# LuletterSoul/RP-Style-Transfer

Measured on AMD Instinct MI355X. Metric: stylized images/sec at 512×512, 1/2/4/8 MI355X; % HBM roofline, higher is better.
Workload: dtype fp32

## Files before the change

### rp-style-transfer_amd/csrc/rpst_conv.h

```cpp
#pragma once

#include "rpst_common.h"

namespace rpst {

constexpr int kTW = 32;

struct ConvArgs {
  const float* in;
  const float* aux;
  const float* aux2;
  const float* wpk;
  const float* bias;
  const float* res;
  float* out;
  int N, Cin, Hs, Ws, H, W, Cout, Cout_pad, nchunks;
  int tiles_x, tiles_y, co_tiles;
  int pad, relu;
  int persist;
  int cosplit;
  float2* stat_part;
  int stat_P;
  int64_t wstride;
  const float* btab;
  int skip_from;
  const float* in2;
  int in2_from;
  const float* mask;
  int pool_out;
};

struct ConvMode {
  int precise;
  int quarter;
  int algo;
  bool narrow;
  int narrow_rpt;
};

struct ConvTiling {
  int64_t blocks;
  int nth;
  int stat_nt, stat_wn, stat_tw;
  bool stat_t;
};

__device__ __forceinline__ const float* conv_in_img(const ConvArgs& a, int n, int64_t per) {
  return (a.in2_from > 0 && n >= a.in2_from) ? a.in2 + (int64_t)(n - a.in2_from) * per
                                             : a.in + (int64_t)n * per;
}

template <int KS>
struct ConvK {
  static constexpr int CK = (KS == 3) ? 8 : 16;
  static constexpr int TAPS = KS * KS;
  static constexpr int KCH = TAPS * CK;
};

__device__ __forceinline__ bool resolve(int& v, int n, int pad, bool padded) {
  if (padded) {
    if (pad == RPST_PAD_ZERO) {
      if (v < 0 || v >= n) return false;
    } else {
      v = reflect1(v, n);
    }
  }
  v = v < 0 ? 0 : (v >= n ? n - 1 : v);
// ... 167 lines not shown
  v += __builtin_bit_cast(float, __builtin_amdgcn_update_dpp(0, __builtin_bit_cast(int, v), 0xB1, 0xF, 0xF, false));
  v += __builtin_bit_cast(float, __builtin_amdgcn_update_dpp(0, __builtin_bit_cast(int, v), 0x4E, 0xF, 0xF, false));
  v += __builtin_bit_cast(float, __builtin_amdgcn_update_dpp(0, __builtin_bit_cast(int, v), 0x141, 0xF, 0xF, false));
  v += __builtin_bit_cast(float, __builtin_amdgcn_update_dpp(0, __builtin_bit_cast(int, v), 0x140, 0xF, 0xF, false));
  return v;
}
__device__ __forceinline__ bool resolve_bf(int& v, int n, bool zero_pad) {
  const bool in = v >= 0 && v < n;
  const int r = reflect1(v, n);
  v = zero_pad ? min(max(v, 0), n - 1) : r;
  return in || !zero_pad;
}
__device__ __forceinline__ void at6(const float (&m)[6], float (&p)[4]) {
  const float s12 = m[1] + m[2], d12 = m[1] - m[2];
  const float s34 = m[3] + m[4], d34 = m[3] - m[4];
  p[0] = (m[0] + s12) + s34;
  p[1] = fmaf(2.f, d34, d12);
  p[2] = fmaf(4.f, s34, s12);
  p[3] = fmaf(8.f, d34, d12) + m[5];
}
__device__ __forceinline__ void w4_tile(int b, int tiles_x, int tiles_y, int& tx, int& ty, int& n) {
  ty = b % tiles_y;
  b /= tiles_y;
  tx = b % tiles_x;
  n = b / tiles_x;
}

bool wino4q_applies(int Cin, int Cout, int in_op, const ConvMode& m);
size_t wino4q_packed_floats(int Cout, int Cin);
int wino4q_pack(const float* w, float* pk, int Cout, int Cin, hipStream_t st);
int wino4q_pack_mix(const double* wm, float* pk, int N, int Cout, int Cin, hipStream_t st);
int wino4q_fold_w(const float* pk, float* out, const float* aux, int N, int Cout, int Cin,
                  hipStream_t st);
ConvTiling wino4q_tiling(ConvArgs& a);
int wino4q_launch(ConvArgs& a, int in_op, hipStream_t st);
inline size_t wino4_image_floats(int Cout, int Cin, bool quarter) {
  return quarter ? wino4q_packed_floats(Cout, Cin) : wino4_packed_floats(Cout, Cin);
}
inline size_t wino4_image_floats_max(int Cout, int Cin) {
  const size_t q = wino4q_packed_floats(Cout, Cin), p = wino4_packed_floats(Cout, Cin);
  return q > p ? q : p;
}

}
```

### rp-style-transfer_amd/csrc/rpst_conv.hip

```cpp
#include "rpst_conv.h"

#include <cstdlib>
#include <cstring>

namespace rpst {

template <int KS, int BM, int TH, int WM, int WN, int INOP, int NTH, int CKK, bool DB>
__global__ __launch_bounds__(NTH, 2) void conv_mfma_kernel(ConvArgs a) {
  using K = ConvK<KS>;
  constexpr int PCK = K::CK, TAPS = K::TAPS;
  constexpr int CK = CKK, KCH = TAPS * CK;
  static_assert(PCK % CK == 0, "kernel chunk must divide the packing chunk");
  constexpr int OFF = (KS == 3) ? 1 : 0;
  constexpr int PH = TH + KS - 1, PW = kTW + KS - 1;
  constexpr int WTM = BM / WM;
  constexpr int MT = WTM / 32;
  constexpr int NT = TH / WN;
  static_assert(WM * WN == NTH / kWave, "one wave per sub-tile");
  static_assert(MT >= 1 && NT >= 1 && (CK % 2) == 0, "tile");
  constexpr int NW4 = KCH * BM / 4;
  constexpr int WLD = (NW4 + NTH - 1) / NTH;
  constexpr bool WFULL = (NW4 % NTH) == 0;
  constexpr int GROUPS = NTH / 32;
  constexpr int CPT = CK > GROUPS ? CK / GROUPS : 1;
// ... 500 lines not shown
  const int wn = bm == 128 ? 2 : 4;
  a.Cout_pad = pad_cout(a.Cout);
  a.nchunks = (a.Cin + ck - 1) / ck;
  a.tiles_x = (a.W + kTW - 1) / kTW;
  a.tiles_y = (a.H + th - 1) / th;
  a.co_tiles = a.Cout_pad / bm;
  a.stat_P = a.tiles_x * a.tiles_y * wn;
  return {(int64_t)a.tiles_x * a.tiles_y * a.N * a.co_tiles, 256, th / wn, wn, kTW, false};
}

static int narrow_rpt(int Cout, const ConvMode& m) {
  return Cout <= 4 && m.narrow_rpt != 2 ? 4 : 2;
}
static ConvTiling narrow_tiling(ConvArgs& a, int rpt) {
  const int rows = 4 * rpt;
  a.Cout_pad = pad_cout(a.Cout);
  a.nchunks = (a.Cin + ConvK<3>::CK - 1) / ConvK<3>::CK;
  a.tiles_x = (a.W + kNrTW - 1) / kNrTW;
  a.tiles_y = (a.H + rows - 1) / rows;
  a.co_tiles = 1;
  a.stat_P = 0;
  return {(int64_t)a.tiles_x * a.tiles_y * a.N, 256, 0, 0, kNrTW, false};
}

static thread_local int t_conv_precise = 0;
static thread_local int t_conv_quarter = -1;

static ConvMode conv_mode() {
  ConvMode m{};
  m.precise = t_conv_precise;
  const char* e = getenv("RPST_W4Q");
  const int q = t_conv_quarter >= 0 ? t_conv_quarter : ((e && *e) ? atoi(e) : 1);
  m.quarter = q == 2 ? 2 : q != 0;
  e = getenv("RPST_CONV_ALGO");
  m.algo = -1;
  if (e && e[0] == 'd') m.algo = RPST_CONV_DIRECT;
  else if (e && !strcmp(e, "winograd")) m.algo = RPST_CONV_WINOGRAD;
  else if (e && !strcmp(e, "winograd4")) m.algo = RPST_CONV_WINOGRAD4;
  e = getenv("RPST_CONV_NARROW");
  m.narrow = !(e && *e && atoi(e) == 0);
  e = getenv("RPST_CONV_NARROW_RPT");
  m.narrow_rpt = (e && *e && atoi(e) == 2) ? 2 : 0;
  return m;
}

static int conv_algo(int Cout, int Cin, int Hs, int Ws, int ksize, int in_op, const ConvMode& m) {
  if (ksize != 3) return RPST_CONV_DIRECT;
  const bool w4 = wino4_supports(in_op) && wino4_fits(1, Cin, Hs, Ws, in_op);
  const bool nr = (in_op == RPST_IN_NONE || (in_op == RPST_IN_ADD_ADAIN && Cout <= 4)) &&
                  narrow_shape(Cin, Cout) && m.narrow;
  if (m.algo == RPST_CONV_DIRECT) return nr ? RPST_CONV_NARROW : RPST_CONV_DIRECT;
  if (m.algo == RPST_CONV_WINOGRAD) return RPST_CONV_WINOGRAD;
  if (m.algo == RPST_CONV_WINOGRAD4) return w4 ? RPST_CONV_WINOGRAD4 : RPST_CONV_WINOGRAD;
  if (nr) return RPST_CONV_NARROW;
  if (Cin <= 4 && w4 && m.precise != 1) return RPST_CONV_WINOGRAD4;
  if (Cin < 16) return RPST_CONV_DIRECT;
  if (w4 && m.precise != 1) return RPST_CONV_WINOGRAD4;
  if (w4) return RPST_CONV_WINOGRAD;
  return Cout >= 32 ? RPST_CONV_WINOGRAD : RPST_CONV_DIRECT;
}

static size_t direct_packed_floats(int Cout, int Cin, int ksize) {
  const int ck = ck_of(ksize);
  const size_t nch = (size_t)(Cin + ck - 1) / ck;
  return nch * ksize * ksize * ck * (size_t)pad_cout(Cout);
}
// ... 16 lines not shown
}

struct ConvNeeds {
  bool stats, residual, fold;
};

struct ConvPlan {
  int algo;
  bool quarter;
  bool fold;
  int op;
  int rpt;
  size_t wofs;
  ConvTiling t;
};

static ConvPlan conv_plan(ConvArgs& a, int ksize, int in_op, const ConvMode& m, ConvNeeds need) {
  ConvPlan p{};
  p.op = in_op;
  p.algo = conv_algo(a.Cout, a.Cin, a.Hs, a.Ws, ksize, in_op, m);
  if (p.algo == RPST_CONV_NARROW) {
    p.rpt = narrow_rpt(a.Cout, m);
    p.t = narrow_tiling(a, p.rpt);
    if (need.stats || a.N > 65535 || a.tiles_y > 65535) p.algo = RPST_CONV_DIRECT;
  }
  if (need.residual && (p.algo == RPST_CONV_WINOGRAD || p.algo == RPST_CONV_WINOGRAD4))
    p.algo = RPST_CONV_DIRECT;
  if (p.algo == RPST_CONV_WINOGRAD4) {
    p.fold = need.fold && !need.stats && a.H >= 2 && a.W >= 2;
    if (p.fold) p.op = RPST_IN_NONE;
    p.quarter = wino4q_applies(a.Cin, a.Cout, p.op, m);
    p.wofs = direct_packed_floats(a.Cout, a.Cin, ksize) + wino_packed_floats(a.Cout, a.Cin) +
             (p.quarter ? wino4_packed_floats(a.Cout, a.Cin) : 0);
    p.t = p.quarter ? wino4q_tiling(a) : wino4_tiling(a);
  } else if (p.algo == RPST_CONV_WINOGRAD) {
    p.wofs = direct_packed_floats(a.Cout, a.Cin, ksize);
    p.t = wino_tiling(a, in_op);
  } else if (p.algo == RPST_CONV_DIRECT) {
    p.t = direct_tiling(a, ksize, in_op);
  }
  return p;
}

template <class F>
static size_t max_over_modes(ConvMode m, F bytes) {
  size_t best = 0;
  for (m.precise = 0; m.precise < 3; ++m.precise)
    for (m.quarter = 0; m.quarter < 3; ++m.quarter) {
      const size_t b = bytes(m);
      best = b > best ? b : best;
    }
  return best;
}

}

using namespace rpst;

extern "C" size_t rpst_conv2d_packed_size(int Cout, int Cin, int ksize) {
  if (Cout <= 0 || Cin <= 0 || (ksize != 1 && ksize != 3)) return 0;
  size_t f = direct_packed_floats(Cout, Cin, ksize);
  if (ksize == 3)
    f += wino_packed_floats(Cout, Cin) + wino4_packed_floats(Cout, Cin) +
         wino4q_packed_floats(Cout, Cin);
  return f * sizeof(float);
}

// ... 124 lines not shown
  a.mask = r.mask;
  a.pool_out = r.pool_out;
  if (r.ksize == 3 && r.pad_mode == RPST_PAD_REFLECT)
    RPST_REQUIRE(a.H >= 2 && a.W >= 2, "conv2d: reflect padding needs H,W >= 2");
  RPST_REQUIRE((int64_t)r.N * (r.Cout > r.Cin ? r.Cout : r.Cin) * a.H * a.W < (1LL << 40),
               "conv2d: tensor too large");
  RPST_REQUIRE(((int64_t)r.Cin + 16) * r.Hs * r.Ws * 4 < (1LL << 31),
               "conv2d: one image's input exceeds 2 GiB");
  const bool fold = r.fold_ws && (r.in_op == RPST_IN_ADAIN || r.T);
  p = conv_plan(a, r.ksize, r.in_op, m, {r.stat_part != nullptr, r.residual != nullptr, fold});
  RPST_REQUIRE(!r.pool_out || p.algo == RPST_CONV_WINOGRAD4,
               "conv2d_pool: the pooled-output epilogue exists on the F(4x4) path only "
               "(rpst_conv2d_algorithm == RPST_CONV_WINOGRAD4)");
  RPST_REQUIRE(!r.T || p.fold, "conv2d_mix: T / offset on a launch that does not fold them");
  a.wpk = r.packed_weight + p.wofs;
  return RPST_OK;
}

template <int KS, int INOP>
static int launch_direct(const ConvArgs& a, hipStream_t st) {
  launch_conv<KS, INOP>(a, direct_bm(a.Cout), st);
  return launch_status("conv_mfma_kernel");
}

static int conv_launch(const ConvReq& r, ConvArgs& a, const ConvPlan& p) {
  hipStream_t st = r.st;
  if (p.algo == RPST_CONV_WINOGRAD4) {
    if (p.fold) {
      const int e = r.T ? wino4_mix(a, p.quarter, r.T, r.offset, r.packed_weight,
                                    pad_cout(r.Cout), r.fold_ws, st)
                        : wino4_fold(a, p.quarter, r.packed_weight, pad_cout(r.Cout), r.fold_ws, st);
      if (e) return e;
    }
    if (int e = p.quarter ? wino4q_launch(a, p.op, st) : wino4_launch(a, p.op, st)) return e;
    if (r.mask) {
      const int64_t n = (int64_t)r.N * r.Cout * a.H * a.W;
      mask_apply_kernel<<<(unsigned)((n + 1023) / 1024), 256, 0, st>>>(r.out, r.mask, n);
      return launch_status("mask_apply_kernel");
    }
    return RPST_OK;
  }
  if (p.algo == RPST_CONV_WINOGRAD) return wino_launch(a, r.in_op, st);
  if (p.algo == RPST_CONV_NARROW) {
    RPST_REQUIRE(r.Cin * 9 * (r.Cout <= 4 ? 4 : 16) <= kNrWl, "conv2d: narrow weights exceed LDS");
    const dim3 grid((unsigned)a.tiles_x, (unsigned)a.tiles_y, r.N);
    if (r.in_op == RPST_IN_ADD_ADAIN) {
      RPST_REQUIRE(r.Cout <= 4, "conv2d: narrow skip-AdaIN conv needs Cout <= 4");
      if (p.rpt == 4) conv3x3_narrow_kernel<4, 4, RPST_IN_ADD_ADAIN><<<grid, 256, 0, st>>>(a);
      else conv3x3_narrow_kernel<4, 2, RPST_IN_ADD_ADAIN><<<grid, 256, 0, st>>>(a);
    } else if (r.Cout <= 4) {
      if (p.rpt == 4) conv3x3_narrow_kernel<4, 4><<<grid, 256, 0, st>>>(a);
      else conv3x3_narrow_kernel<4, 2><<<grid, 256, 0, st>>>(a);
    } else {
      conv3x3_narrow_kernel<16, 2><<<grid, 256, 0, st>>>(a);
    }
    return launch_status("conv3x3_narrow_kernel");
  }
  RPST_REQUIRE(p.t.blocks <= 0x7fffffffLL, "conv2d: grid too large");
  if (r.ksize == 1) {
    RPST_REQUIRE(r.in_op == RPST_IN_NONE, "conv2d: 1x1 conv supports in_op NONE only");
    return launch_direct<1, RPST_IN_NONE>(a, st);
  }
  switch (r.in_op) {
    case RPST_IN_MAXPOOL2: return launch_direct<3, RPST_IN_MAXPOOL2>(a, st);
    case RPST_IN_UPSAMPLE2: return launch_direct<3, RPST_IN_UPSAMPLE2>(a, st);
    case RPST_IN_ADD_UPSAMPLE2: return launch_direct<3, RPST_IN_ADD_UPSAMPLE2>(a, st);
    case RPST_IN_ADAIN: return launch_direct<3, RPST_IN_ADAIN>(a, st);
// ... 315 lines not shown
```

### rp-style-transfer_amd/csrc/rpst_wino4q.hip

```cpp
#include "rpst_conv.h"

#include <type_traits>

#ifndef RPST_W4Q_DBG
#define RPST_W4Q_DBG 0
#endif

namespace rpst {
namespace {

template <int PAD>
__device__ __forceinline__ void q_mfma(floatx4& acc, float a, float b) {
  if constexpr (PAD)
    asm volatile("s_nop 1\n\tv_mfma_f32_16x16x4_f32 %0, %1, %2, %0" : "+v"(acc) : "v"(a), "v"(b));
  else
    asm volatile("v_mfma_f32_16x16x4_f32 %0, %1, %2, %0" : "+v"(acc) : "v"(a), "v"(b));
}
__device__ __forceinline__ unsigned q_lds_addr(const float* p) {
  return (unsigned)(uintptr_t)(const __attribute__((address_space(3))) float*)p;
}
template <int OFF>
__device__ __forceinline__ void q_dma16(__amdgpu_buffer_rsrc_t r, unsigned m0, unsigned voff,
                                        int soff) {
  asm volatile("s_mov_b32 m0, %0\n\ts_nop 0\n\tbuffer_load_dwordx4 %1, %2, %3 offen offset:%4 lds"
// ... 14 lines not shown
                                      float& u0, float& u1, float& u2) {
  if constexpr (H == 0) {
    const float A = fmaf(-4.f, d2, d4), B = fmaf(-4.f, d1, d3);
    u0 = fmaf(4.f, d0, fmaf(-5.f, d2, d4));
    u1 = A + B;
    u2 = A - B;
  } else {
    const float C = d4 - d2, E = d3 - d1;
    u0 = fmaf(2.f, E, C);
    u1 = fmaf(-2.f, E, C);
    u2 = fmaf(4.f, d1, fmaf(-5.f, d3, d5));
  }
}

}

constexpr int kQCo = 64;
constexpr int kQTH = 8, kQTW = 64;
constexpr int kQXO = 4;
constexpr int kQPS = 72;
constexpr int kQCS = 768;
constexpr int kQWS = 9216;
constexpr int kQPAT = 4 * kQCS;
constexpr int kQNTH = 512;
constexpr int kQMaxCo = 512;
constexpr int kQWPI = 5;
constexpr int kQWide = 2, kQSlow = 6;
constexpr int kQDMA4 = 3, kQDMA = 12;
constexpr int kQRP = kQPS / 4;
constexpr int kQXS = 4 * 3 * 3 * 64 * 2;
constexpr int kQWG0 = 0;
constexpr int kQPG = 5;
constexpr int kQAhead = 3;
static_assert(10 * kQRP <= kQDMA4 * 64 && kQDMA4 * 256 <= kQCS, "16-B pieces in a channel");
static_assert(10 * kQPS <= kQDMA * 64 && kQDMA * 64 <= kQCS, "4-B pieces in a channel");
static_assert(2 * kQWide >= kQDMA4 && 2 * kQSlow >= kQDMA && 8 * kQWPI >= 36, "coverage");
static_assert(2 * kQXS <= kQWS, "the exchange fits a weight stage");
static_assert((2 * kQWS + 4 * kQPAT) * 4 + 1024 + kQSlow * kQNTH * 4 + 9 * kQMaxCo * 4 <= 163840,
              "LDS");

template <typename TW>
__global__ void wino4q_pack_kernel(const TW* __restrict__ w, float* __restrict__ pk, int Cout,
                                   int Cin, int K4, int64_t per, int64_t total, int64_t sco,
                                   int64_t sci, int64_t stap) {
  int64_t t = (int64_t)blockIdx.x * blockDim.x + threadIdx.x;
  if (t >= total) return;
  const int64_t img = t / per;
  pk += img * per;
  w += img * (int64_t)Cout * Cin * 9;
  t -= img * per;
  const int cb = (int)(t & 3);
  int64_t r = t >> 2;
  const int l = (int)(r & 63);
  r >>= 6;
  const int p = (int)(r % 9);
  r /= 9;
  const int q = (int)(r & 3);
  r >>= 2;
  const int ks = (int)(r % K4);
  const int ct = (int)(r / K4);
  const int i = 3 * (q >> 1) + p / 3, jj = 3 * (q & 1) + p % 3;
  const int co = ct * kQCo + cb * 16 + (l & 15);
  const int ci = ks * 4 + (l >> 4);
  float v = 0.f;
  if (co < Cout && ci < Cin) {
    const double G[6][3] = {{0.25, 0, 0},
// ... 33 lines not shown

__global__ void wino4q_fold_w_kernel(const float4* __restrict__ pk, float4* __restrict__ out,
                                     const float* __restrict__ aux, int N, int Cin, int K4,
                                     int64_t per4) {
  const int64_t t = (int64_t)blockIdx.x * blockDim.x + threadIdx.x;
  if (t >= (int64_t)N * per4) return;
  const int n = (int)(t / per4);
  const int64_t u = t - (int64_t)n * per4;
  const int l = (int)(u & 63);
  const int ks = (int)((u / (kQWS / 4)) % K4);
  const int ci = ks * 4 + (l >> 4);
  const int64_t nc = (int64_t)N * Cin, i = (int64_t)n * Cin + (ci < Cin ? ci : 0);
  const float sc = ci < Cin ? aux[3 * nc + i] / aux[2 * nc + i] : 0.f;
  const float4 v = pk[u];
  out[t] = make_float4(v.x * sc, v.y * sc, v.z * sc, v.w * sc);
}

int wino4q_fold_w(const float* pk, float* out, const float* aux, int N, int Cout, int Cin,
                  hipStream_t st) {
  const int64_t per4 = (int64_t)wino4q_packed_floats(Cout, Cin) / 4, n4 = (int64_t)N * per4;
  wino4q_fold_w_kernel<<<(unsigned)((n4 + 255) / 256), 256, 0, st>>>(
      reinterpret_cast<const float4*>(pk), reinterpret_cast<float4*>(out), aux, N, Cin,
      (Cin + 3) / 4, per4);
  return launch_status("wino4q_fold_w_kernel");
}

bool wino4q_applies(int Cin, int Cout, int in_op, const ConvMode& m) {
  const int min_cin = m.quarter == 2 ? 16 : 128;
  return m.quarter && m.precise != 2 && (in_op == RPST_IN_NONE || in_op == RPST_IN_UPSAMPLE2) &&
         Cout >= 64 && Cout <= kQMaxCo &&
         Cin >= min_cin && Cin % 16 == 0;
}

ConvTiling wino4q_tiling(ConvArgs& a) {
  a.Cout_pad = (a.Cout + kQCo - 1) / kQCo * kQCo;
  a.nchunks = (a.Cin + 3) / 4;
  a.tiles_x = (a.W + kQTW - 1) / kQTW;
  a.tiles_y = (a.H + kQTH - 1) / kQTH;
  a.co_tiles = a.Cout_pad / kQCo;
  a.stat_P = a.tiles_x * a.tiles_y * 2;
  a.cosplit = 1;
  return {(int64_t)a.tiles_x * a.tiles_y * a.N, kQNTH, 4, kQTH / 4, kQTW, true};
}

struct QEpi {
  int W, H, Cout, gy0, gx0, rows, n, sidx;
  bool vec, full, bst, edge, store, pool;
  float inv, slope;
  unsigned voff[4];
  float* out;
  float* oimg;
  unsigned obytes;
  const float* btab;
  float2* statp;
  int statP;
};

__device__ __forceinline__ QEpi q_epi_ctx(int wr, int tn) {
  const KArgs L = late_args();
  QEpi e;
  e.W = L->W;
  e.H = L->H;
  e.Cout = L->Cout;
  e.slope = L->relu == RPST_ACT_RELU ? 0.f : (L->relu == RPST_ACT_LRELU ? 0.2f : 1.f);
  int btx, bty;
  w4_tile((int)blockIdx.x / L->cosplit, L->tiles_x, L->tiles_y, btx, bty, e.n);
  const int bx0 = btx * kQTW;
  e.gy0 = bty * kQTH + 4 * wr;
  e.gx0 = bx0 + 4 * tn;
  e.vec = (e.W & 3) == 0 && e.gx0 + 3 < e.W;
  e.rows = max(0, min(4, e.H - e.gy0));
  const int cols = max(0, min(kQTW, e.W - bx0));
  e.inv = e.rows * cols > 0 ? __builtin_amdgcn_rcpf((float)(e.rows * cols)) : 0.f;
  e.full = e.rows == 4 && bx0 + kQTW <= e.W;
  e.edge = e.gy0 == 0 || e.gy0 + 4 >= e.H || bx0 == 0 || bx0 + kQTW >= e.W;
  e.out = L->out;
  const int64_t plane = (int64_t)e.H * e.W;
  e.pool = L->pool_out != 0;
  e.bst = !e.pool && (e.W & 3) == 0 && (int64_t)e.Cout * plane * 4 < (1LL << 31);
  e.oimg = e.out + (int64_t)e.n * e.Cout * plane;
  const bool keep = L->skip_from <= 0 || e.n < L->skip_from;
  e.obytes = keep ? (unsigned)(e.Cout * plane * 4) : 0u;
  e.store = keep;
#pragma unroll
  for (int yy = 0; yy < 4; ++yy)
    e.voff[yy] = (yy < e.rows && e.gx0 < e.W) ? (unsigned)(((e.gy0 + yy) * e.W + e.gx0) * 4)
                                             : 0x80000000u;
  e.btab = L->btab;
  e.statp = L->stat_part;
  e.statP = L->stat_P;
  e.sidx = (bty * L->tiles_x + btx) * 2 + wr;
  return e;
}

template <bool STATS, bool BTAB, bool RELU>
__device__ __forceinline__ void q_finish(const QEpi& e, int co, float (&Y)[16], int tn) {
  const int gy0 = e.gy0, gx0 = e.gx0, rows = e.rows, n = e.n;
  const bool cok = co < e.Cout;
  if constexpr (BTAB) {
// ... 96 lines not shown
#pragma unroll
      for (int i = 0; i < 16; ++i) m2 = fmaf(Y[i] - mean, Y[i] - mean, m2);
    } else {
#pragma unroll
      for (int yy = 0; yy < 4; ++yy)
#pragma unroll
        for (int xx = 0; xx < 4; ++xx) {
          const float dv = Y[yy * 4 + xx] - mean;
          m2 += (yy < rows && gx0 + xx < e.W) ? dv * dv : 0.f;
        }
    }
    m2 = row16_sum(m2);
    if (tn == 0 && cok)
      e.statp[((int64_t)n * e.statP + e.sidx) * e.Cout + co] = make_float2(mean, m2);
  }
}

template <int INOP, bool STATS, bool BTAB, bool RELU>
__global__ __launch_bounds__(kQNTH, 1) void wino4q_mfma_kernel(ConvArgs a) {
  __shared__ __attribute__((aligned(16))) float ws0[kQWS];
  __shared__ __attribute__((aligned(16))) float ws1[kQWS];
  __shared__ __attribute__((aligned(16))) float ps0[kQPAT];
  __shared__ __attribute__((aligned(16))) float ps1[kQPAT];
  __shared__ __attribute__((aligned(16))) float ps2[kQPAT];
  __shared__ __attribute__((aligned(16))) float ps3[kQPAT];
  __shared__ __attribute__((aligned(16))) float dummy[256];
  __shared__ unsigned poffs[kQSlow][kQNTH];
  __shared__ float btl[BTAB ? 9 * kQMaxCo : kQMaxCo];

  const int wave = __builtin_amdgcn_readfirstlane((int)threadIdx.x >> 6);
  const int lane = threadIdx.x & 63;
  const int k = lane >> 4, tn = lane & 15, wr = wave >> 2;

  int bid = (int)blockIdx.x;
  const int cog = bid % a.cosplit;
  bid /= a.cosplit;
  const int nct = a.co_tiles / a.cosplit, ct0 = cog * nct;
  int tx, ty, n;
  w4_tile(bid, a.tiles_x, a.tiles_y, tx, ty, n);
  const int K4 = a.nchunks, G = nct * K4;
  const int y0 = ty * kQTH, x0 = tx * kQTW;

  {
    const int nb = BTAB ? 9 * a.Cout : a.Cout;
    const float* src = BTAB ? a.btab + (int64_t)n * nb : a.bias;
    for (int i = threadIdx.x; i < nb; i += kQNTH) btl[i] = src ? src[i] : 0.f;
  }
  constexpr bool up = INOP == RPST_IN_UPSAMPLE2;
  const unsigned in_plane = up ? (unsigned)(a.Hs * a.Ws) : (unsigned)(a.H * a.W);
  const unsigned oob = a.Cin * in_plane * 4u;
  const float* in_img = conv_in_img(a, n, (int64_t)a.Cin * in_plane);
  const unsigned wbytes = (unsigned)(nct * K4 * kQWS) * 4u;
  const float* w_img = a.wpk + (int64_t)n * a.wstride + (int64_t)ct0 * K4 * kQWS;

  const int hf = wave & 1;
  const bool zp = a.pad == RPST_PAD_ZERO;
  const int rs = up ? a.Ws : a.W;
  const bool w4a = (a.W & 3) == 0;
  const bool wide = !up && ((x0 >= 1 && x0 + kQTW < a.W) || (w4a && x0 + kQTW <= a.W));
  const bool fixL = wide && w4a && !zp && x0 == 0;
  const bool fixR = wide && w4a && !zp && x0 + kQTW == a.W;
  unsigned poff[kQSlow];
  const int tid = threadIdx.x;
  if (wide) {
#pragma unroll
    for (int i = 0; i < kQWide; ++i) {
      const int p = kQWide * hf + i;
      const int f = 64 * p + lane, row = min(f / kQRP, 9), j = f - (f / kQRP) * kQRP;
      int y = y0 - 1 + row;
      const int xs = x0 - kQXO + 4 * j;
      const bool okx = !w4a || (xs >= 0 && xs + 3 < a.W);
      const bool ok = p < kQDMA4 && f < 10 * kQRP && resolve_bf(y, a.H, zp) && okx;
      poff[i] = ok ? ((unsigned)(y * rs) + (unsigned)xs) * 4u : oob;
    }
#pragma unroll
    for (int i = kQWide; i < kQSlow; ++i) poff[i] = oob;
  } else {
#pragma unroll
    for (int i = 0; i < kQSlow; ++i) {
      const int p = kQSlow * hf + i;
      const int f = 64 * p + lane;
      const int row = min(f / kQPS, 9), col = f - (f / kQPS) * kQPS;
      int y = y0 - 1 + row, x = x0 - kQXO + col;
      const bool oky = resolve_bf(y, a.H, zp), okx = resolve_bf(x, a.W, zp);
      const bool ok = p < kQDMA && col >= kQXO - 1 && col < kQXO + 1 + kQTW &&
                      f < 10 * kQPS && oky && okx;
      poff[i] = ok ? ((unsigned)((up ? y >> 1 : y) * rs) + (unsigned)(up ? x >> 1 : x)) * 4u : oob;
    }
  }
#pragma unroll
  for (int i = 0; i < kQSlow; ++i) poffs[i][tid] = poff[i];

  constexpr int DBG = RPST_W4Q_DBG;
  const int wl = wave * 4096;
  const bool real4 = wave < 4;
  const int w4 = 32768 + wave * 1024;
  const unsigned dummy_a = q_lds_addr(dummy);
  int wso = wl;
  auto issue_w = [&](bool live, unsigned stg, auto Ic) {
    constexpr int I = decltype(Ic)::value;
    if (DBG & 2) return;
    if constexpr (I < 4) {
      q_dma16<1024 * I>(rsrc_or_zero(w_img, wbytes, live), stg + wl, lane * 16, wso);
    } else {
      q_dma16<0>(rsrc_or_zero(w_img, wbytes, live && real4), real4 ? stg + w4 : dummy_a,
                 lane * 16, wso + (w4 - wl));
    }
  };
  const unsigned pstep = 4u * in_plane * 4u;
  const int pbase = (int)((unsigned)(wave >> 1) * in_plane * 4u);
  const bool h1 = (wave & 1) != 0;
  const int pl = (wave >> 1) * (kQCS * 4) + (h1 ? (wide ? 2048 : kQSlow * 256) : 0);
  int pso = pbase;
  auto issue_p = [&](auto WIDEc, bool live, unsigned stg) {
    constexpr bool WIDE = decltype(WIDEc)::value;
    if (DBG & 1) return;
    const auto r = rsrc_or_zero(in_img, oob, live);
    const unsigned xs = stg + launder(pl);
    if constexpr (WIDE) {
      q_dma16<0>(r, xs, poffs[0][tid], pso);
      q_dma16<0>(r, h1 ? dummy_a : xs + 1024, poffs[1][tid], pso);
    } else {
#pragma unroll
      for (int i = 0; i < kQSlow; ++i) q_dma4(r, xs + 256 * i, poffs[i][tid], pso);
    }
    pso += (int)pstep;
  };
  const bool bst_all = !a.pool_out && (a.W & 3) == 0 &&
                       (int64_t)a.Cout * a.H * a.W * 4 < (1LL << 31);
  bool post_epi = false;
  auto wait_ring = [&](bool first) {
    if (DBG & 128) return;
    if (first && post_epi && bst_all) {
      if (wide) asm volatile("s_waitcnt vmcnt(18)" ::: "memory");
      else asm volatile("s_waitcnt vmcnt(22)" ::: "memory");
    } else if (wide) {
      asm volatile("s_waitcnt vmcnt(2)" ::: "memory");
    } else {
      asm volatile("s_waitcnt vmcnt(6)" ::: "memory");
    }
    if (first) post_epi = false;
  };

  auto fix_halo = [&](float* stg) {
    if ((wave == 0 && fixL) || (wave == 1 && fixR)) {
      int l = lane;
      asm volatile("" : "+v"(l));
      if (l < 40) {
        const int ch = l / 10, row = l - 10 * ch;
        float* rp = stg + ch * kQCS + row * kQPS;
        if (wave == 0) rp[kQXO - 1] = rp[kQXO + 1];
        else rp[kQXO + kQTW] = rp[kQXO + kQTW - 2];
      }
    }
  };
  auto prologue = [&](auto WIDEc) {
    issue_p(WIDEc, true, q_lds_addr(ps0));
    issue_p(WIDEc, true, q_lds_addr(ps1));
    issue_w(true, q_lds_addr(ws0), std::integral_constant<int, 0>{});
    issue_w(true, q_lds_addr(ws0), std::integral_constant<int, 1>{});
    issue_w(true, q_lds_addr(ws0), std::integral_constant<int, 2>{});
    issue_w(true, q_lds_addr(ws0), std::integral_constant<int, 3>{});
    issue_w(true, q_lds_addr(ws0), std::integral_constant<int, 4>{});
    issue_p(WIDEc, true, q_lds_addr(ps2));
    issue_p(WIDEc, true, q_lds_addr(ps3));
  };
  if (wide) prologue(std::true_type{});
  else prologue(std::false_type{});
  wait_ring(false);
  q_lds_barrier();
  if (fixL || fixR) {
    fix_halo(ps0);
    fix_halo(ps1);
    q_lds_barrier();
  }

  auto body = [&](auto Qc) {
    constexpr int Q = decltype(Qc)::value, QR = Q >> 1, QC = Q & 1;
    floatx4 acc[9][4];
#pragma unroll
    for (int p = 0; p < 9; ++p)
#pragma unroll
      for (int cb = 0; cb < 4; ++cb) acc[p][cb] = floatx4{0.f, 0.f, 0.f, 0.f};
    const int roff = k * kQCS + (4 * wr + QR) * kQPS + 4 * tn;
    auto read_row = [&](const float* stg, int rr, float (&d)[8]) {
      const float* rp = stg + roff + rr * kQPS;
      floatx4 u = *reinterpret_cast<const floatx4*>(rp + 4);
      const float e = QC ? rp[8] : rp[3];
      asm("" : "+v"(u));
      d[0] = QC ? 0.f : e; d[1] = u[0]; d[2] = u[1]; d[3] = u[2]; d[4] = u[3];
      d[5] = QC ? e : 0.f; d[6] = 0.f; d[7] = 0.f;
    };
    auto col_pass = [&](const float (&d)[8], float (&u)[3]) {
      if (DBG & 8) {
        u[0] = d[0]; u[1] = d[1]; u[2] = d[2];
        return;
      }
      q_bt3<QC>(d[0], d[1], d[2], d[3], d[4], d[5], u[0], u[1], u[2]);
    };
    auto row_pass = [&](const float (&u)[5][3], int j, float (&v)[9]) {
      if (DBG & 8) {
        v[j] = u[0][j]; v[3 + j] = u[2][j]; v[6 + j] = u[4][j];
        return;
      }
      if constexpr (QR == 0)
        q_bt3<0>(u[0][j], u[1][j], u[2][j], u[3][j], u[4][j], 0.f, v[j], v[3 + j], v[6 + j]);
      else
        q_bt3<1>(0.f, u[0][j], u[1][j], u[2][j], u[3][j], u[4][j], v[j], v[3 + j], v[6 + j]);
    };
    float V[9];
    {
      float u[5][3];
#pragma unroll
      for (int rr = 0; rr < 5; ++rr) {
        float d[8];
        read_row(ps0, rr, d);
        col_pass(d, u[rr]);
      }
#pragma unroll
      for (int j = 0; j < 3; ++j) row_pass(u, j, V);
    }

    const int woff = Q * 9 * 256 + lane * 4;
    int x = 0;
    auto step = [&](float* wsx, float* psn, float* wsn, float* psx, float* pfx, int ks,
                    bool first) {
      wait_ring(first);
      const bool wlive = x + 1 < G, plive = x + 4 < G;
      wso += kQWS * 4;
      if (first && ks + 4 == K4) pso = pbase;
      const unsigned wsn_a = q_lds_addr(wsn), psx_a = q_lds_addr(psx);
      if (DBG & 16) asm volatile("s_waitcnt lgkmcnt(0)" ::: "memory");
      else q_lds_barrier();
      constexpr int ord[9] = {0, 3, 6, 1, 4, 7, 2, 5, 8};
      constexpr int kA = kQAhead;
      float4 w4[9];
#pragma unroll
      for (int q = 0; q < kA; ++q)
        w4[ord[q]] = *reinterpret_cast<const float4*>(wsx + woff + ord[q] * 256);
      float d[8];
      read_row(psn, 0, d);
      float u[5][3];
#pragma unroll
      for (int q = 0; q < 9; ++q) {
        const int p = ord[q];
        if (q + kA < 9)
          w4[ord[q + kA]] = *reinterpret_cast<const float4*>(wsx + woff + ord[q + kA] * 256);
        q_mfma<1>(acc[p][0], w4[p].x, V[p]);
        q_mfma<0>(acc[p][1], w4[p].y, V[p]);
        q_mfma<0>(acc[p][2], w4[p].z, V[p]);
        q_mfma<0>(acc[p][3], w4[p].w, V[p]);
        if (q == kQWG0) issue_w(wlive, wsn_a, std::integral_constant<int, 0>{});
        if (q == kQWG0 + 1) issue_w(wlive, wsn_a, std::integral_constant<int, 1>{});
        if (q == kQWG0 + 2) issue_w(wlive, wsn_a, std::integral_constant<int, 2>{});
        if (q == kQWG0 + 3) issue_w(wlive, wsn_a, std::integral_constant<int, 3>{});
        if (q == kQWG0 + 4) issue_w(wlive, wsn_a, std::integral_constant<int, 4>{});
        if (q == kQPG) {
          if (wide) issue_p(std::true_type{}, plive, psx_a);
          else issue_p(std::false_type{}, plive, psx_a);
        }
        if (q < 5) {
          col_pass(d, u[q]);
          if (q + 1 < 5) read_row(psn, q + 1, d);
        }
        if (q == 5 || q == 6 || q == 8) row_pass(u, q == 8 ? 2 : q - 5, V);
        if (q == 7) fix_halo(pfx);
      }
      ++x;
    };

    auto epilogue = [&](int ctile) {
      if (DBG & 32) {
        float t = 0.f;
#pragma unroll
        for (int p = 0; p < 9; ++p)
#pragma unroll
          for (int cb = 0; cb < 4; ++cb) t += acc[p][cb][0];
        if (t == 1.2345f) late_args()->out[threadIdx.x] = t;
#pragma unroll
        for (int p = 0; p < 9; ++p)
#pragma unroll
          for (int cb = 0; cb < 4; ++cb) acc[p][cb] = floatx4{0.f, 0.f, 0.f, 0.f};
        return;
      }
      q_lds_barrier();
      asm volatile("s_nop 7\n\ts_nop 4" : "+v"(acc[0][0]), "+v"(acc[0][1]), "+v"(acc[0][2]),
                   "+v"(acc[0][3]), "+v"(acc[1][0]), "+v"(acc[1][1]), "+v"(acc[1][2]),
                   "+v"(acc[1][3]), "+v"(acc[2][0]), "+v"(acc[2][1]), "+v"(acc[2][2]),
                   "+v"(acc[2][3]), "+v"(acc[3][0]), "+v"(acc[3][1]), "+v"(acc[3][2]),
                   "+v"(acc[3][3]), "+v"(acc[4][0]), "+v"(acc[4][1]));
      asm volatile("" : "+v"(acc[4][2]), "+v"(acc[4][3]), "+v"(acc[5][0]), "+v"(acc[5][1]),
                   "+v"(acc[5][2]), "+v"(acc[5][3]), "+v"(acc[6][0]), "+v"(acc[6][1]),
                   "+v"(acc[6][2]), "+v"(acc[6][3]), "+v"(acc[7][0]), "+v"(acc[7][1]),
                   "+v"(acc[7][2]), "+v"(acc[7][3]), "+v"(acc[8][0]), "+v"(acc[8][1]),
                   "+v"(acc[8][2]), "+v"(acc[8][3]));
      const int co0 = ctile * kQCo + 16 * Q + 4 * k;
#pragma unroll
      for (int rp = 0; rp < 2; ++rp) {
        float P[2][6][4];
// ... 7 lines not shown
#pragma unroll
            for (int j = 0; j < 3; ++j)
              *reinterpret_cast<float2*>(xb + (((dq * 3 + slot) * 3 + j) * 64 + lane) * 2) =
                  make_float2(acc[3 * pt + j][dq][2 * rp], acc[3 * pt + j][dq][2 * rp + 1]);
          }
          if (!(DBG & 4)) q_lds_barrier();
          float m[2][2][6];
#pragma unroll
          for (int s = 0; s < 4; ++s) {
#pragma unroll
            for (int j = 0; j < 3; ++j) {
              float2 v;
              if (s == Q || (DBG & 4)) {
                const int src = (DBG & 4) ? s : Q;
                v = make_float2(acc[3 * pt + j][src][2 * rp], acc[3 * pt + j][src][2 * rp + 1]);
              } else {
                v = *reinterpret_cast<const float2*>(
                    xb + (((Q * 3 + ((s - Q - 1) & 3)) * 3 + j) * 64 + lane) * 2);
              }
              m[0][s >> 1][3 * (s & 1) + j] = v.x;
              m[1][s >> 1][3 * (s & 1) + j] = v.y;
            }
          }
#pragma unroll
          for (int e2 = 0; e2 < 2; ++e2) {
            at6(m[e2][0], P[e2][pt]);
            at6(m[e2][1], P[e2][3 + pt]);
          }
          if (!(DBG & 4) && (rp == 0 || pt < 2)) q_lds_barrier();
        }
#pragma unroll
        for (int e2 = 0; e2 < 2; ++e2) {
          const int r = 2 * rp + e2;
          QEpi e = q_epi_ctx(wr, tn);
          e.btab = btl;
          float bias = 0.f;
          {
            const int co = co0 + r;
            if (co < e.Cout) bias = BTAB ? btl[co * 9 + 4] : btl[co];
          }
#pragma unroll
          for (int x = 0; x < 4; ++x) P[e2][1][x] += bias;
          float Y[16];
#pragma unroll
          for (int x = 0; x < 4; ++x) {
            float c6[6], y[4];
#pragma unroll
            for (int I = 0; I < 6; ++I) c6[I] = P[e2][I][x];
            at6(c6, y);
#pragma unroll
            for (int yy = 0; yy < 4; ++yy) Y[yy * 4 + x] = y[yy];
          }
          q_finish<STATS, BTAB, RELU>(e, co0 + r, Y, tn);
        }
      }
#pragma unroll
      for (int p = 0; p < 9; ++p)
#pragma unroll
        for (int cb = 0; cb < 4; ++cb) acc[p][cb] = floatx4{0.f, 0.f, 0.f, 0.f};
    };

    int ks = 0, ct = ct0;
    for (int g = 0; g < G; g += 4) {
      step(ws0, ps1, ws1, ps0, ps2, ks, true);
      step(ws1, ps2, ws0, ps1, ps3, ks + 1, false);
      step(ws0, ps3, ws1, ps2, ps0, ks + 2, false);
      step(ws1, ps0, ws0, ps3, ps1, ks + 3, false);
      ks += 4;
      if (ks == K4) {
        epilogue(ct);
        post_epi = true;
        ks = 0;
        ++ct;
      }
    }
  };
  switch (wave & 3) {
    case 0: body(std::integral_constant<int, 0>{}); break;
    case 1: body(std::integral_constant<int, 1>{}); break;
    case 2: body(std::integral_constant<int, 2>{}); break;
    default: body(std::integral_constant<int, 3>{}); break;
  }
  asm volatile("s_waitcnt vmcnt(0)" ::: "memory");
}

int wino4q_launch(ConvArgs& a, int in_op, hipStream_t st) {
  RPST_REQUIRE(in_op == RPST_IN_NONE || in_op == RPST_IN_UPSAMPLE2,
               "conv2d: winograd4 (quarter) does not support in_op %d", in_op);
  const ConvTiling t = wino4q_tiling(a);
  RPST_REQUIRE((int64_t)a.co_tiles * a.nchunks * kQWS * 4 < (1LL << 31),
               "conv2d: winograd4 weight image exceeds 2 GiB");
  RPST_REQUIRE(t.blocks <= 0x7fffffffLL, "conv2d: grid too large");
  const unsigned nb = (unsigned)t.blocks;
  const bool stats = a.stat_part != nullptr, btab = a.btab != nullptr;
  RPST_REQUIRE(!btab || in_op == RPST_IN_NONE, "conv2d: winograd4 bias table with a loader op");
  RPST_REQUIRE(!(stats && btab), "conv2d: winograd4 folded bias with statistics");
#define RPST_W4Q_GO(OP, S, B)                                                  \
  do {                                                                         \
    if (a.relu == RPST_ACT_RELU)                                               \
      wino4q_mfma_kernel<OP, S, B, true><<<nb, kQNTH, 0, st>>>(a);             \
    else                                                                       \
      wino4q_mfma_kernel<OP, S, B, false><<<nb, kQNTH, 0, st>>>(a);            \
  } while (0)
  if (in_op == RPST_IN_UPSAMPLE2) {
    if (stats) RPST_W4Q_GO(RPST_IN_UPSAMPLE2, true, false);
    else RPST_W4Q_GO(RPST_IN_UPSAMPLE2, false, false);
  } else {
    if (stats) RPST_W4Q_GO(RPST_IN_NONE, true, false);
    else if (btab) RPST_W4Q_GO(RPST_IN_NONE, false, true);
    else RPST_W4Q_GO(RPST_IN_NONE, false, false);
  }
#undef RPST_W4Q_GO
  return launch_status("wino4q_mfma_kernel");
}

}
```

Baseline: 571.0.

## Make quarter-Winograd conv kernel persistent over a capped grid of tiles

The quarter-precision Winograd-4 conv kernel now launches at most 256 blocks (overridable via RPST_W4Q_BLOCKS), and each block loops over spatial tiles with stride gridDim. The next tile's patch offsets, weight image pointer and bias table are prepared inside the pipelined main loop so the software pipeline continues across tile boundaries. The cosplit output-channel splitting path is dropped. The aim is to cut per-block launch, prologue and pipeline-fill overhead, at the cost of more complex control flow and possible load imbalance or lower occupancy on small workloads.

```diff
diff --git a/rp-style-transfer_amd/csrc/rpst_conv.h b/rp-style-transfer_amd/csrc/rpst_conv.h
--- a/rp-style-transfer_amd/csrc/rpst_conv.h
+++ b/rp-style-transfer_amd/csrc/rpst_conv.h
@@ -33,6 +33,7 @@
 struct ConvMode {
   int precise;
   int quarter;
+  int w4q_blocks;
   int algo;
   bool narrow;
   int narrow_rpt;
@@ -266,8 +267,8 @@
 int wino4q_pack_mix(const double* wm, float* pk, int N, int Cout, int Cin, hipStream_t st);
 int wino4q_fold_w(const float* pk, float* out, const float* aux, int N, int Cout, int Cin,
                   hipStream_t st);
-ConvTiling wino4q_tiling(ConvArgs& a);
-int wino4q_launch(ConvArgs& a, int in_op, hipStream_t st);
+ConvTiling wino4q_tiling(ConvArgs& a, int cap);
+int wino4q_launch(ConvArgs& a, int in_op, int cap, hipStream_t st);
 inline size_t wino4_image_floats(int Cout, int Cin, bool quarter) {
   return quarter ? wino4q_packed_floats(Cout, Cin) : wino4_packed_floats(Cout, Cin);
 }
diff --git a/rp-style-transfer_amd/csrc/rpst_conv.hip b/rp-style-transfer_amd/csrc/rpst_conv.hip
--- a/rp-style-transfer_amd/csrc/rpst_conv.hip
+++ b/rp-style-transfer_amd/csrc/rpst_conv.hip
@@ -556,6 +556,8 @@
   const char* e = getenv("RPST_W4Q");
   const int q = t_conv_quarter >= 0 ? t_conv_quarter : ((e && *e) ? atoi(e) : 1);
   m.quarter = q == 2 ? 2 : q != 0;
+  e = getenv("RPST_W4Q_BLOCKS");
+  m.w4q_blocks = (e && *e) ? atoi(e) : 0;
   e = getenv("RPST_CONV_ALGO");
   m.algo = -1;
   if (e && e[0] == 'd') m.algo = RPST_CONV_DIRECT;
@@ -638,7 +640,7 @@
     p.quarter = wino4q_applies(a.Cin, a.Cout, p.op, m);
     p.wofs = direct_packed_floats(a.Cout, a.Cin, ksize) + wino_packed_floats(a.Cout, a.Cin) +
              (p.quarter ? wino4_packed_floats(a.Cout, a.Cin) : 0);
-    p.t = p.quarter ? wino4q_tiling(a) : wino4_tiling(a);
+    p.t = p.quarter ? wino4q_tiling(a, m.w4q_blocks) : wino4_tiling(a);
   } else if (p.algo == RPST_CONV_WINOGRAD) {
     p.wofs = direct_packed_floats(a.Cout, a.Cin, ksize);
     p.t = wino_tiling(a, in_op);
@@ -829,7 +831,8 @@
                         : wino4_fold(a, p.quarter, r.packed_weight, pad_cout(r.Cout), r.fold_ws, st);
       if (e) return e;
     }
-    if (int e = p.quarter ? wino4q_launch(a, p.op, st) : wino4_launch(a, p.op, st)) return e;
+    if (int e = p.quarter ? wino4q_launch(a, p.op, (int)p.t.blocks, st) : wino4_launch(a, p.op, st))
+      return e;
     if (r.mask) {
       const int64_t n = (int64_t)r.N * r.Cout * a.H * a.W;
       mask_apply_kernel<<<(unsigned)((n + 1023) / 1024), 256, 0, st>>>(r.out, r.mask, n);
diff --git a/rp-style-transfer_amd/csrc/rpst_wino4q.hip b/rp-style-transfer_amd/csrc/rpst_wino4q.hip
--- a/rp-style-transfer_amd/csrc/rpst_wino4q.hip
+++ b/rp-style-transfer_amd/csrc/rpst_wino4q.hip
@@ -70,6 +70,8 @@
 constexpr int kQWG0 = 0;
 constexpr int kQPG = 5;
 constexpr int kQAhead = 3;
+constexpr int kQBlocks = 256;
+static_assert(kQBlocks % 8 == 0 && (9 * kQMaxCo) % 64 == 0, "XCD classes; bias-table pieces");
 static_assert(10 * kQRP <= kQDMA4 * 64 && kQDMA4 * 256 <= kQCS, "16-B pieces in a channel");
 static_assert(10 * kQPS <= kQDMA * 64 && kQDMA * 64 <= kQCS, "4-B pieces in a channel");
 static_assert(2 * kQWide >= kQDMA4 && 2 * kQSlow >= kQDMA && 8 * kQWPI >= 36, "coverage");
@@ -169,7 +171,7 @@
          Cin >= min_cin && Cin % 16 == 0;
 }
 
-ConvTiling wino4q_tiling(ConvArgs& a) {
+ConvTiling wino4q_tiling(ConvArgs& a, int cap) {
   a.Cout_pad = (a.Cout + kQCo - 1) / kQCo * kQCo;
   a.nchunks = (a.Cin + 3) / 4;
   a.tiles_x = (a.W + kQTW - 1) / kQTW;
@@ -177,7 +179,9 @@
   a.co_tiles = a.Cout_pad / kQCo;
   a.stat_P = a.tiles_x * a.tiles_y * 2;
   a.cosplit = 1;
-  return {(int64_t)a.tiles_x * a.tiles_y * a.N, kQNTH, 4, kQTH / 4, kQTW, true};
+  const int64_t tiles = (int64_t)a.tiles_x * a.tiles_y * a.N;
+  const int64_t most = cap > 0 ? cap : kQBlocks;
+  return {tiles < most ? tiles : most, kQNTH, 4, kQTH / 4, kQTW, true};
 }
 
 struct QEpi {
@@ -193,7 +197,7 @@
   int statP;
 };
 
-__device__ __forceinline__ QEpi q_epi_ctx(int wr, int tn) {
+__device__ __forceinline__ QEpi q_epi_ctx(int wr, int tn, int tile) {
   const KArgs L = late_args();
   QEpi e;
   e.W = L->W;
@@ -201,7 +205,7 @@
   e.Cout = L->Cout;
   e.slope = L->relu == RPST_ACT_RELU ? 0.f : (L->relu == RPST_ACT_LRELU ? 0.2f : 1.f);
   int btx, bty;
-  w4_tile((int)blockIdx.x / L->cosplit, L->tiles_x, L->tiles_y, btx, bty, e.n);
+  w4_tile(tile, L->tiles_x, L->tiles_y, btx, bty, e.n);
   const int bx0 = btx * kQTW;
   e.gy0 = bty * kQTH + 4 * wr;
   e.gx0 = bx0 + 4 * tn;
@@ -364,64 +368,92 @@
   const int lane = threadIdx.x & 63;
   const int k = lane >> 4, tn = lane & 15, wr = wave >> 2;
 
-  int bid = (int)blockIdx.x;
-  const int cog = bid % a.cosplit;
-  bid /= a.cosplit;
-  const int nct = a.co_tiles / a.cosplit, ct0 = cog * nct;
-  int tx, ty, n;
-  w4_tile(bid, a.tiles_x, a.tiles_y, tx, ty, n);
-  const int K4 = a.nchunks, G = nct * K4;
-  const int y0 = ty * kQTH, x0 = tx * kQTW;
+  const int nblk = (int)gridDim.x;
+  int tc = (int)blockIdx.x;
+  const int K4 = a.nchunks, GT = a.co_tiles * K4;
+  const int G = (a.tiles_x * a.tiles_y * a.N - tc + nblk - 1) / nblk * GT;
+  int n_c;
+  {
+    int tx, ty;
+    w4_tile(tc, a.tiles_x, a.tiles_y, tx, ty, n_c);
+  }
 
   {
     const int nb = BTAB ? 9 * a.Cout : a.Cout;
-    const float* src = BTAB ? a.btab + (int64_t)n * nb : a.bias;
+    const float* src = BTAB ? a.btab + (int64_t)n_c * nb : a.bias;
     for (int i = threadIdx.x; i < nb; i += kQNTH) btl[i] = src ? src[i] : 0.f;
   }
   constexpr bool up = INOP == RPST_IN_UPSAMPLE2;
   const unsigned in_plane = up ? (unsigned)(a.Hs * a.Ws) : (unsigned)(a.H * a.W);
   const unsigned oob = a.Cin * in_plane * 4u;
-  const float* in_img = conv_in_img(a, n, (int64_t)a.Cin * in_plane);
-  const unsigned wbytes = (unsigned)(nct * K4 * kQWS) * 4u;
-  const float* w_img = a.wpk + (int64_t)n * a.wstride + (int64_t)ct0 * K4 * kQWS;
+  const unsigned wbytes = (unsigned)(GT * kQWS) * 4u;
+  const float* w_img = a.wpk + (int64_t)n_c * a.wstride;
 
   const int hf = wave & 1;
-  const bool zp = a.pad == RPST_PAD_ZERO;
-  const int rs = up ? a.Ws : a.W;
-  const bool w4a = (a.W & 3) == 0;
-  const bool wide = !up && ((x0 >= 1 && x0 + kQTW < a.W) || (w4a && x0 + kQTW <= a.W));
-  const bool fixL = wide && w4a && !zp && x0 == 0;
-  const bool fixR = wide && w4a && !zp && x0 + kQTW == a.W;
-  unsigned poff[kQSlow];
+  const bool h1 = hf != 0;
   const int tid = threadIdx.x;
-  if (wide) {
-#pragma unroll
-    for (int i = 0; i < kQWide; ++i) {
-      const int p = kQWide * hf + i;
-      const int f = 64 * p + lane, row = min(f / kQRP, 9), j = f - (f / kQRP) * kQRP;
-      int y = y0 - 1 + row;
-      const int xs = x0 - kQXO + 4 * j;
-      const bool okx = !w4a || (xs >= 0 && xs + 3 < a.W);
-      const bool ok = p < kQDMA4 && f < 10 * kQRP && resolve_bf(y, a.H, zp) && okx;
-      poff[i] = ok ? ((unsigned)(y * rs) + (unsigned)xs) * 4u : oob;
-    }
-#pragma unroll
-    for (int i = kQWide; i < kQSlow; ++i) poff[i] = oob;
-  } else {
-#pragma unroll
-    for (int i = 0; i < kQSlow; ++i) {
-      const int p = kQSlow * hf + i;
-      const int f = 64 * p + lane;
-      const int row = min(f / kQPS, 9), col = f - (f / kQPS) * kQPS;
-      int y = y0 - 1 + row, x = x0 - kQXO + col;
-      const bool oky = resolve_bf(y, a.H, zp), okx = resolve_bf(x, a.W, zp);
-      const bool ok = p < kQDMA && col >= kQXO - 1 && col < kQXO + 1 + kQTW &&
-                      f < 10 * kQPS && oky && okx;
-      poff[i] = ok ? ((unsigned)((up ? y >> 1 : y) * rs) + (unsigned)(up ? x >> 1 : x)) * 4u : oob;
-    }
-  }
-#pragma unroll
-  for (int i = 0; i < kQSlow; ++i) poffs[i][tid] = poff[i];
+  const float* in_img;
+  int pl, pf = 0;
+  constexpr int kFWide = 1, kFFix = 2, kFRefill = 4, kFWideC = 16, kFFixC = 32;
+  auto patch_tile = [&](int tile) -> bool {
+    const KArgs L = late_args();
+    int ln = lane;
+    asm volatile("" : "+v"(ln));
+    const int hw = launder(hf);
+    const int H = L->H, W = L->W;
+    int tx, ty, n;
+    w4_tile(tile, L->tiles_x, L->tiles_y, tx, ty, n);
+    const int y0 = ty * kQTH, x0 = tx * kQTW;
+    const unsigned plane = up ? (unsigned)(L->Hs * L->Ws) : (unsigned)(H * W);
+    const unsigned oobp = L->Cin * plane * 4u;
+    const int64_t per = (int64_t)L->Cin * plane;
+    const int in2_from = L->in2_from;
+    in_img = (in2_from > 0 && n >= in2_from) ? L->in2 + (int64_t)(n - in2_from) * per
+                                             : L->in + (int64_t)n * per;
+    const bool zp = L->pad == RPST_PAD_ZERO;
+    const int rs = up ? L->Ws : W;
+    const bool w4a = (W & 3) == 0;
+    const bool wide = !up && ((x0 >= 1 && x0 + kQTW < W) || (w4a && x0 + kQTW <= W));
+    const bool fixL = wide && w4a && !zp && x0 == 0;
+    const bool fixR = wide && w4a && !zp && x0 + kQTW == W;
+    pf = launder(__builtin_amdgcn_readfirstlane(
+        (pf & ~(kFWide | kFFix)) | (wide ? kFWide : 0) |
+        ((wave == 0 ? fixL : (wave == 1 && fixR)) ? kFFix : 0)));
+    pl = (wave >> 1) * (kQCS * 4) + (h1 ? (wide ? 2048 : kQSlow * 256) : 0);
+    unsigned poff[kQSlow];
+    if (wide) {
+#pragma unroll
+      for (int i = 0; i < kQWide; ++i) {
+        const int p = kQWide * hw + i;
+        const int f = 64 * p + ln, row = min(f / kQRP, 9), j = f - (f / kQRP) * kQRP;
+        int y = y0 - 1 + row;
+        const int xs = x0 - kQXO + 4 * j;
+        const bool okx = !w4a || (xs >= 0 && xs + 3 < W);
+        const bool ok = p < kQDMA4 && f < 10 * kQRP && resolve_bf(y, H, zp) && okx;
+        poff[i] = ok ? ((unsigned)(y * rs) + (unsigned)xs) * 4u : oobp;
+      }
+#pragma unroll
+      for (int i = kQWide; i < kQSlow; ++i) poff[i] = oobp;
+    } else {
+#pragma unroll
+      for (int i = 0; i < kQSlow; ++i) {
+        const int p = kQSlow * hw + i;
+        const int f = 64 * p + ln;
+        const int row = min(f / kQPS, 9), col = f - (f / kQPS) * kQPS;
+        int y = y0 - 1 + row, x = x0 - kQXO + col;
+        const bool oky = resolve_bf(y, H, zp), okx = resolve_bf(x, W, zp);
+        const bool ok = p < kQDMA && col >= kQXO - 1 && col < kQXO + 1 + kQTW &&
+                        f < 10 * kQPS && oky && okx;
+        poff[i] =
+            ok ? ((unsigned)((up ? y >> 1 : y) * rs) + (unsigned)(up ? x >> 1 : x)) * 4u : oobp;
+      }
+    }
+#pragma unroll
+    for (int i = 0; i < kQSlow; ++i) poffs[i][tid] = poff[i];
+    return fixL || fixR;
+  };
+  const bool fix0 = patch_tile(tc);
+  pf |= pf << 4;
 
   constexpr int DBG = RPST_W4Q_DBG;
   const int wl = wave * 4096;
@@ -441,8 +473,6 @@
   };
   const unsigned pstep = 4u * in_plane * 4u;
   const int pbase = (int)((unsigned)(wave >> 1) * in_plane * 4u);
-  const bool h1 = (wave & 1) != 0;
-  const int pl = (wave >> 1) * (kQCS * 4) + (h1 ? (wide ? 2048 : kQSlow * 256) : 0);
   int pso = pbase;
   auto issue_p = [&](auto WIDEc, bool live, unsigned stg) {
     constexpr bool WIDE = decltype(WIDEc)::value;
@@ -461,7 +491,7 @@
   const bool bst_all = !a.pool_out && (a.W & 3) == 0 &&
                        (int64_t)a.Cout * a.H * a.W * 4 < (1LL << 31);
   bool post_epi = false;
-  auto wait_ring = [&](bool first) {
+  auto wait_ring = [&](bool first, bool wide) {
     if (DBG & 128) return;
     if (first && post_epi && bst_all) {
       if (wide) asm volatile("s_waitcnt vmcnt(18)" ::: "memory");
@@ -474,8 +504,8 @@
     if (first) post_epi = false;
   };
 
-  auto fix_halo = [&](float* stg) {
-    if ((wave == 0 && fixL) || (wave == 1 && fixR)) {
+  auto fix_halo = [&](float* stg, bool mine) {
+    if (mine) {
       int l = lane;
       asm volatile("" : "+v"(l));
       if (l < 40) {
@@ -497,15 +527,22 @@
     issue_p(WIDEc, true, q_lds_addr(ps2));
     issue_p(WIDEc, true, q_lds_addr(ps3));
   };
-  if (wide) prologue(std::true_type{});
+  if (pf & kFWide) prologue(std::true_type{});
   else prologue(std::false_type{});
-  wait_ring(false);
+  wait_ring(false, (pf & kFWide) != 0);
   q_lds_barrier();
-  if (fixL || fixR) {
-    fix_halo(ps0);
-    fix_halo(ps1);
+  if (fix0) {
+    fix_halo(ps0, (pf & kFFix) != 0);
+    fix_halo(ps1, (pf & kFFix) != 0);
     q_lds_barrier();
   }
+  auto refill_btl = [&]() {
+    const KArgs L = late_args();
+    const int nbt = 9 * L->Cout;
+    const auto r = rsrc_or_zero(L->btab + (int64_t)n_c * nbt, (unsigned)nbt * 4u, true);
+    const unsigned btl_a = q_lds_addr(btl);
+    for (int p = wave; p * 64 < nbt; p += 8) q_dma4(r, btl_a + 256 * p, 256 * p + lane * 4, 0);
+  };
 
   auto body = [&](auto Qc) {
     constexpr int Q = decltype(Qc)::value, QR = Q >> 1, QC = Q & 1;
@@ -555,15 +592,21 @@
 
     const int woff = Q * 9 * 256 + lane * 4;
     int x = 0;
-    auto step = [&](float* wsx, float* psn, float* wsn, float* psx, float* pfx, int ks,
-                    bool first) {
-      wait_ring(first);
+    auto step = [&](float* wsx, float* psn, float* wsn, float* psx, float* pfx, auto Jc) {
+      constexpr int J = decltype(Jc)::value;
+      constexpr bool first = J == 0;
+      wait_ring(first, (pf & (J == 0 ? kFWideC : kFWide)) != 0);
       const bool wlive = x + 1 < G, plive = x + 4 < G;
       wso += kQWS * 4;
-      if (first && ks + 4 == K4) pso = pbase;
       const unsigned wsn_a = q_lds_addr(wsn), psx_a = q_lds_addr(psx);
       if (DBG & 16) asm volatile("s_waitcnt lgkmcnt(0)" ::: "memory");
       else q_lds_barrier();
+      if constexpr (BTAB && first) {
+        if (pf & kFRefill) {
+          refill_btl();
+          pf &= ~kFRefill;
+        }
+      }
       constexpr int ord[9] = {0, 3, 6, 1, 4, 7, 2, 5, 8};
       constexpr int kA = kQAhead;
       float4 w4[9];
@@ -588,7 +631,7 @@
         if (q == kQWG0 + 3) issue_w(wlive, wsn_a, std::integral_constant<int, 3>{});
         if (q == kQWG0 + 4) issue_w(wlive, wsn_a, std::integral_constant<int, 4>{});
         if (q == kQPG) {
-          if (wide) issue_p(std::true_type{}, plive, psx_a);
+          if (pf & kFWide) issue_p(std::true_type{}, plive, psx_a);
           else issue_p(std::false_type{}, plive, psx_a);
         }
         if (q < 5) {
@@ -596,7 +639,7 @@
           if (q + 1 < 5) read_row(psn, q + 1, d);
         }
         if (q == 5 || q == 6 || q == 8) row_pass(u, q == 8 ? 2 : q - 5, V);
-        if (q == 7) fix_halo(pfx);
+        if (q == 7) fix_halo(pfx, (pf & (J >= 2 ? kFFix : kFFixC)) != 0);
       }
       ++x;
     };
@@ -670,7 +713,7 @@
 #pragma unroll
         for (int e2 = 0; e2 < 2; ++e2) {
           const int r = 2 * rp + e2;
-          QEpi e = q_epi_ctx(wr, tn);
+          QEpi e = q_epi_ctx(wr, tn, tc);
           e.btab = btl;
           float bias = 0.f;
           {
@@ -698,12 +741,24 @@
         for (int cb = 0; cb < 4; ++cb) acc[p][cb] = floatx4{0.f, 0.f, 0.f, 0.f};
     };
 
-    int ks = 0, ct = ct0;
+    int ks = 0, ct = 0;
+    int rem = GT >> 2;
     for (int g = 0; g < G; g += 4) {
-      step(ws0, ps1, ws1, ps0, ps2, ks, true);
-      step(ws1, ps2, ws0, ps1, ps3, ks + 1, false);
-      step(ws0, ps3, ws1, ps2, ps0, ks + 2, false);
-      step(ws1, ps0, ws0, ps3, ps1, ks + 3, false);
+      if (ks + 4 == K4) {
+        pso = pbase;
+        if (rem == 1 && g + 4 < G) patch_tile(tc + nblk);
+      }
+      step(ws0, ps1, ws1, ps0, ps2, std::integral_constant<int, 0>{});
+      step(ws1, ps2, ws0, ps1, ps3, std::integral_constant<int, 1>{});
+      step(ws0, ps3, ws1, ps2, ps0, std::integral_constant<int, 2>{});
+      if (rem == 1) {
+        const KArgs L = late_args();
+        int tx, ty, n;
+        w4_tile(tc + nblk, L->tiles_x, L->tiles_y, tx, ty, n);
+        w_img = L->wpk + (int64_t)n * L->wstride;
+        wso = wl - kQWS * 4;
+      }
+      step(ws1, ps0, ws0, ps3, ps1, std::integral_constant<int, 3>{});
       ks += 4;
       if (ks == K4) {
         epilogue(ct);
@@ -711,6 +766,19 @@
         ks = 0;
         ++ct;
       }
+      if (--rem == 0) {
+        const KArgs L = late_args();
+        rem = (L->co_tiles * L->nchunks) >> 2;
+        ct = 0;
+        tc += nblk;
+        pf = (pf & (kFWide | kFFix)) * 17;
+        if constexpr (BTAB) {
+          int tx, ty, n;
+          w4_tile(tc, L->tiles_x, L->tiles_y, tx, ty, n);
+          if (n != n_c) pf |= kFRefill;
+          n_c = n;
+        }
+      }
     }
   };
   switch (wave & 3) {
@@ -722,10 +790,11 @@
   asm volatile("s_waitcnt vmcnt(0)" ::: "memory");
 }
 
-int wino4q_launch(ConvArgs& a, int in_op, hipStream_t st) {
+int wino4q_launch(ConvArgs& a, int in_op, int cap, hipStream_t st) {
   RPST_REQUIRE(in_op == RPST_IN_NONE || in_op == RPST_IN_UPSAMPLE2,
                "conv2d: winograd4 (quarter) does not support in_op %d", in_op);
-  const ConvTiling t = wino4q_tiling(a);
+  const ConvTiling t = wino4q_tiling(a, cap);
+  RPST_REQUIRE((int64_t)a.tiles_x * a.tiles_y * a.N <= 0x7fffffffLL, "conv2d: too many tiles");
   RPST_REQUIRE((int64_t)a.co_tiles * a.nchunks * kQWS * 4 < (1LL << 31),
                "conv2d: winograd4 weight image exceeds 2 GiB");
   RPST_REQUIRE(t.blocks <= 0x7fffffffLL, "conv2d: grid too large");
```

Result: no change. 574.3, median of 6 (+0.6%).
